# custom-computing-ic/TRPO-Robot-Control

Hardware: AMD Instinct MI355X
Metric: FVP samples/sec + 10-iter CG wall time, armDOF_0 policy (higher is better)
Workload: dtype fp32; 1 GPU; cg10_armDOF_0_N50000; policy=armDOF_0 [15,16,16,3] lttl, samples=50000, samples_per_rank=50000, cg_iters=10, parallelism=dp1 (contiguous sample shards, peer-window all-reduce per FVP), cg_scalars=fp64, fvp_kernel=mfma-mlp3 1x1x1x1 ttl no-mfma

## Files before the change

### trpo-robot-control_amd/csrc/trpo_kernels.hip

```cpp
#include <hip/hip_runtime.h>
#include <rccl/rccl.h>

#include <dlfcn.h>
#include <math.h>
#include <pthread.h>
#include <stdarg.h>
#include <stdint.h>
#include <stdio.h>
#include <stdlib.h>
#include <string.h>
#include <time.h>

#include "trpo_common.h"
#include "trpo_dev.h"

typedef float f4 __attribute__((ext_vector_type(4)));

#define MFMA(a, b, c) __builtin_amdgcn_mfma_f32_16x16x4f32((a), (b), (c), 0, 0, 0)
#define MFMA4(a, b, c) __builtin_amdgcn_mfma_f32_4x4x1f32((a), (b), (c), 0, 0, 0)

struct Pack {
    int T[4];
    int fa[3], fb[3], bi[3], iv, tlen;
    int vfa[3], vb[3], vlen;
// ... 437 lines not shown
            const int a = w / lo, o = w - a * lo;
            const int lane = (o & 15) + 16 * ((a & 15) >> 2);
            return vfa[i] + (((o >> 4) * T[i] + (a >> 4)) * 64 + lane) * 4 + (a & 3);
        }
        if (b >= 0 && b < lo) return vb[i] + b;
    }
    return -1;
}

__device__ __forceinline__ int imap_at(const Net &n, const int (&T)[4], int j) {
    const int k = j >> 8, lane = (j >> 2) & 63, r = j & 3, c = lane & 15, g = lane >> 4;
    int base = 0;
#pragma unroll
    for (int i = 0; i < 3; ++i) {
        const int nt = T[i] * T[i + 1];
        if (k >= base && k < base + nt) {
            const int at = (k - base) / T[i + 1], bt = (k - base) % T[i + 1];
            const int a = 16 * at + 4 * g + r, b = 16 * bt + c;
            return (a < n.L[i] && b < n.L[i + 1]) ? n.woff[i] + a * n.L[i + 1] + b : -1;
        }
        base += nt;
    }
#pragma unroll
    for (int i = 0; i < 3; ++i) {
        if (k >= base && k < base + T[i + 1]) {
            const int b = 16 * (k - base) + 4 * g + r;
            return (c == 0 && b < n.L[i + 1]) ? n.boff[i] + b : -1;
        }
        base += T[i + 1];
    }
    return -1;
}

__device__ __forceinline__ int islot_at(const Net &n, const int (&T)[4], int q) {
    int kw[3], kb[3], k = 0;
#pragma unroll
    for (int i = 0; i < 3; ++i) { kw[i] = k; k += T[i] * T[i + 1]; }
#pragma unroll
    for (int i = 0; i < 3; ++i) { kb[i] = k; k += T[i + 1]; }
#pragma unroll
    for (int i = 0; i < 3; ++i) {
        const int lo = n.L[i + 1], w = q - n.woff[i], b = q - n.boff[i];
        if (w >= 0 && w < n.L[i] * lo) {
            const int a = w / lo, o = w - a * lo;
            return (kw[i] + (a >> 4) * T[i + 1] + (o >> 4)) * 256 + (((a & 15) >> 2) * 16 + (o & 15)) * 4 + (a & 3);
        }
        if (b >= 0 && b < lo) return (kb[i] + (b >> 4)) * 256 + ((b & 15) >> 2) * 64 + (b & 3);
    }
    return -1;
}

__global__ void build_maps_kernel(Net n, Pack pk, int *tmap, int *vmap, int p64) {
    const int e = blockIdx.x * blockDim.x + threadIdx.x;
    if (e < pk.tlen) {
        int m = -1;
        for (int i = 0; i < 3; ++i) {
            if (e >= pk.fa[i] && e < pk.fa[i] + 256 * pk.T[i] * pk.T[i + 1])
                m = map_frag(n, i, e - pk.fa[i], pk.T[i], true, p64 != 0);
            if (i > 0 && e >= pk.fb[i] && e < pk.fb[i] + 256 * pk.T[i] * pk.T[i + 1])
                m = map_frag(n, i, e - pk.fb[i], pk.T[i + 1], false, p64 != 0);
            if (e >= pk.bi[i] && e < pk.bi[i] + 16 * pk.T[i + 1]) {
                const int j = e - pk.bi[i];
                m = j < n.L[i + 1] ? n.boff[i] + j : -1;
            }
        }
        tmap[e] = m;
    }
    if (e < pk.vlen) vmap[e] = vmap_at(n, pk.T, e, p64 != 0);
}

__global__ void build_pslot_kernel(Net n, Pack pk, int *ps, int P) {
    const int q = blockIdx.x * blockDim.x + threadIdx.x;
    const int T[4] = {pk.T[0], pk.T[1], pk.T[2], pk.T[3]};
    if (q < P) ps[q] = pslot_at(n, T, q);
}
__global__ void build_islot_kernel(Net n, Pack pk, int *is, int nw) {
    const int q = blockIdx.x * blockDim.x + threadIdx.x;
    const int T[4] = {pk.T[0], pk.T[1], pk.T[2], pk.T[3]};
    if (q < nw) is[q] = islot_at(n, T, q);
}

__global__ void gather_pack_kernel(void *dst, const double *src, const int *map, int len, int f64) {
    const int e = blockIdx.x * blockDim.x + threadIdx.x;
    if (e < len) {
        const int m = map[e];
        const double v = m >= 0 ? src[m] : 0.0;
        if (f64) reinterpret_cast<double *>(dst)[e] = v;
        else reinterpret_cast<float *>(dst)[e] = (float)v;
    }
}

__global__ void build_imap_kernel(Net n, Pack pk, int *imap, int slab) {
    const int j = blockIdx.x * blockDim.x + threadIdx.x;
    if (j < slab) imap[j] = imap_at(n, pk.T, j);
}

__global__ void iota_kernel(int *v, int len, int valid) {
    const int j = blockIdx.x * blockDim.x + threadIdx.x;
    if (j < len) v[j] = j < valid ? j : -1;
}

__global__ void set_invvar_kernel(void *iv, const double *stdv, int A, int len, int f64) {
    const int j = blockIdx.x * blockDim.x + threadIdx.x;
    if (j < len) {
        const double v = j < A ? 1.0 / stdv[j] / stdv[j] : 0.0;
        if (f64) reinterpret_cast<double *>(iv)[j] = v;
        else reinterpret_cast<float *>(iv)[j] = (float)v;
    }
}

__global__ void obs_pad_kernel(void *dst, const double *src, int n, int npad, int L0, int ld, int f64) {
    const long e = (long)blockIdx.x * blockDim.x + threadIdx.x;
    if (e >= (long)npad * ld) return;
    const int s = (int)(e / ld), k = (int)(e % ld);
    const int q = k & 15, kf = f64 ? (k - q) + (q >> 2) + 4 * (q & 3) : k;
    const double v = (s < n && kf < L0) ? src[(long)s * L0 + kf] : 0.0;
    if (f64) reinterpret_cast<double *>(dst)[e] = v;
    else reinterpret_cast<float *>(dst)[e] = (float)v;
}

__global__ void to_f32_kernel(float *dst, const double *src, int len) {
    const int e = blockIdx.x * blockDim.x + threadIdx.x;
    if (e < len) dst[e] = (float)src[e];
}
__global__ void to_elem_kernel(void *dst, const double *src, long len, int f64) {
    const long e = (long)blockIdx.x * blockDim.x + threadIdx.x;
    if (e >= len) return;
    if (f64) reinterpret_cast<double *>(dst)[e] = src[e];
    else reinterpret_cast<float *>(dst)[e] = (float)src[e];
}


constexpr int SCR_LD = 20;

template <int T0, int T1, int T2, int T3>
struct FastCfg {
    static constexpr int FA0 = 0;
    static constexpr int FA1 = FA0 + 256 * T0 * T1;
    static constexpr int FA2 = FA1 + 256 * T1 * T2;
    static constexpr int FB1 = FA2 + 256 * T2 * T3;
    static constexpr int FB2 = FB1 + 256 * T1 * T2;
    static constexpr int BI0 = FB2 + 256 * T2 * T3;
    static constexpr int BI1 = BI0 + 16 * T1;
    static constexpr int BI2 = BI1 + 16 * T2;
    static constexpr int IV = BI2 + 16 * T3;
    static constexpr int TLEN = IV + 16 * T3;
    static constexpr int VFA0 = 0;
    static constexpr int VFA1 = VFA0 + 256 * T0 * T1;
    static constexpr int VFA2 = VFA1 + 256 * T1 * T2;
    static constexpr int VB0 = VFA2 + 256 * T2 * T3;
    static constexpr int VB1 = VB0 + 16 * T1;
    static constexpr int VB2 = VB1 + 16 * T2;
    static constexpr int VLEN = VB2 + 16 * T3;
    static constexpr int R0 = 16 * (T0 + T1), R1 = 16 * (T1 + T2), R2 = 16 * (T2 + T3);
    static constexpr int ROWS = R0 > R1 ? (R0 > R2 ? R0 : R2) : (R1 > R2 ? R1 : R2);
    static constexpr int SCR = ROWS * 20;
    static constexpr int NACC = 4 * (T0 * T1 + T1 * T2 + T2 * T3 + T1 + T2 + T3);
    static constexpr int SLAB = NACC * 64;
    static constexpr bool REGW = T0 * T1 + T1 * T2 + T2 * T3 <= 3;
    static constexpr int WAVES = 8;
    static constexpr int NT_YC = 1;
    static constexpr int THREADS = 64 * WAVES;
    static constexpr int PMAX = 256 * (T0 * T1 + T1 * T2 + T2 * T3) + 16 * (T1 + T2 + 2 * T3);
    static constexpr int SCRATCH = (WAVES * NT_YC * SCR > 2 * PMAX) ? WAVES * NT_YC * SCR : 2 * PMAX;
    static constexpr int MAIN_BYTES = 4 * (TLEN + VLEN + SCRATCH);
    static constexpr int CAP = MAIN_BYTES > 131072 ? MAIN_BYTES : 131072;
    static constexpr int rw_pick(int w) {
        return w < 1 ? 1 : ((WAVES % w == 0 && w * SLAB * 4 <= CAP) ? w : rw_pick(w - 1));
    }
    static constexpr int RW = rw_pick(WAVES);
    static constexpr int EPT = (SLAB / 4 + THREADS - 1) / THREADS;
    static constexpr int EMAX = (PMAX + THREADS - 1) / THREADS;
    static constexpr int VEMAX = (VLEN + THREADS - 1) / THREADS;
    static constexpr int EMAX_REPLICAS = 4;
    static_assert(NT_YC == 1 || NT_YC == 2, "NT");
    static_assert(WAVES % RW == 0, "RW");
    static int lds_bytes() {
        const int b = 4 * RW * SLAB;
        return MAIN_BYTES > b ? MAIN_BYTES : b;
    }
};

__device__ __forceinline__ float rowsum16(float v) {
    int x = __float_as_int(v);
    v += __int_as_float(__builtin_amdgcn_update_dpp(0, x, 0xB1, 0xF, 0xF, false));
    x = __float_as_int(v);
    v += __int_as_float(__builtin_amdgcn_update_dpp(0, x, 0x4E, 0xF, 0xF, false));
    x = __float_as_int(v);
    v += __int_as_float(__builtin_amdgcn_update_dpp(0, x, 0x124, 0xF, 0xF, false));
    x = __float_as_int(v);
    v += __int_as_float(__builtin_amdgcn_update_dpp(0, x, 0x128, 0xF, 0xF, false));
    return v;
}

__device__ __forceinline__ float rowgroup_sum(float v) {
    const auto h = __builtin_amdgcn_permlane32_swap(__float_as_uint(v), __float_as_uint(v), false, false);
    const float t = __uint_as_float(h[0]) + __uint_as_float(h[1]);
    const auto q = __builtin_amdgcn_permlane16_swap(__float_as_uint(t), __float_as_uint(t), false, false);
    return __uint_as_float(q[0]) + __uint_as_float(q[1]);
}
__device__ __forceinline__ f4 rowgroup_sum4(f4 v) {
    const auto p01 = __builtin_amdgcn_permlane32_swap(__float_as_uint(v[0]), __float_as_uint(v[1]), false, false);
    const auto p23 = __builtin_amdgcn_permlane32_swap(__float_as_uint(v[2]), __float_as_uint(v[3]), false, false);
    const float s01 = __uint_as_float(p01[0]) + __uint_as_float(p01[1]);
    const float s23 = __uint_as_float(p23[0]) + __uint_as_float(p23[1]);
    const auto q = __builtin_amdgcn_permlane16_swap(__float_as_uint(s01), __float_as_uint(s23), false, false);
    const float t = __uint_as_float(q[0]) + __uint_as_float(q[1]);
    const auto h = __builtin_amdgcn_permlane32_swap(__float_as_uint(t), __float_as_uint(t), false, false);
    const auto b02 = __builtin_amdgcn_permlane16_swap(h[0], h[0], false, false);
    const auto b13 = __builtin_amdgcn_permlane16_swap(h[1], h[1], false, false);
    f4 r;
    r[0] = __uint_as_float(b02[0]);
    r[1] = __uint_as_float(b13[0]);
    r[2] = __uint_as_float(b02[1]);
    r[3] = __uint_as_float(b13[1]);
    return r;
}

__device__ __forceinline__ f4 stream_ld(const f4 *p) {
    return *p;
}

__device__ __forceinline__ int scr_off(int row, int chunk) {
    const int q = (row >> 2) & 3;
    return row * 16 + (row >> 2) * 16 + ((chunk ^ ((4 - q) & 3)) << 2);
}
__device__ __forceinline__ void scr_put(float *scr, int row0, f4 t, int c, int g) {
    reinterpret_cast<f4 *>(scr)[(row0 >> 4) * 68 + c + 17 * g] = t;
}
__device__ __forceinline__ f4 scr_get(const float *scr, int row0, int c, int g) {
    const float *p = scr + (row0 >> 4) * 272 + 4 * (4 * g + 17 * (c >> 2)) + (c & 3);
    f4 r;
    r[0] = p[0];
    r[1] = p[4];
    r[2] = p[8];
    r[3] = p[12];
    return r;
}

constexpr int NO_MFMA_RGW2 = 8;
template <int T0, int T1, int T2, int T3, int ACT, int MODE, int QB = 0, int NO = 0>
__global__ void __launch_bounds__((64 * FastCfg<T0, T1, T2, T3>::WAVES))
fvp_mlp3_kernel(const double *__restrict__ k_acc, const double *__restrict__ k_p, const double *__restrict__ k_r,
                const double *__restrict__ k_x, const int *__restrict__ k_pslot, const void *k_q, int k_meta,
                IterArgs A, Net net) {
    constexpr bool FV = MODE != 1;
    constexpr bool YC = MODE == 2 || MODE == 3;
    constexpr int NYC = T1 + T2 + T3;
    using C = FastCfg<T0, T1, T2, T3>;
    constexpr int NT = YC ? C::NT_YC : 1;
    static_assert(!YC || C::REGW, "forward cache only for the small-net kernels");
    extern __shared__ __attribute__((aligned(16))) float lds[];
    __shared__ double sh64[(5 + QB) * 4 * C::WAVES];
    double *shq = reinterpret_cast<double *>(lds + C::TLEN + C::VLEN);
    float *qf = reinterpret_cast<float *>(A.q);
    const float *qfz = reinterpret_cast<const float *>(A.qz);
    const int kPs = k_meta & 0xFFFFF, kR = (k_meta >> 20) & 63, knq = (k_meta >> 26) & 63;
    const float *kq = reinterpret_cast<const float *>(k_q);
    static_assert(C::SCRATCH >= 2 * QCAP * 4 * C::WAVES, "basis-dot scratch");
    float *tw = lds;
    float *vw = lds + C::TLEN;
    const int tid = threadIdx.x, lane = tid & 63, wave = tid >> 6;
    const int c = lane & 15, g = lane >> 4;
    float *scr = lds + C::TLEN + C::VLEN + wave * C::NT_YC * C::SCR;
    const int nwaves = gridDim.x * C::WAVES;
    const int ntiles = A.ntiles, n = A.n;
    const f4 *obs4 = reinterpret_cast<const f4 *>(A.obs4);

    constexpr bool CGK = MODE == 3;
    const bool upd = CGK || (MODE == 0 && A.update != 0);
    const bool ini = !CGK && MODE == 0 && !upd && A.init != 0;
    const bool vnat = !CGK && !upd && !ini && A.v_nat != nullptr;
    constexpr int NT4 = C::TLEN / 4, NALL = CGK ? NT4 : (C::TLEN + C::VLEN) / 4;
    constexpr int PER = (NALL + C::THREADS - 1) / C::THREADS;
    const int skipv = *A.skip;
    f4 st[PER];
    int tile = __builtin_amdgcn_readfirstlane(blockIdx.x * C::WAVES + wave);
    constexpr bool RING = YC;
    constexpr int PFU = RING ? 2 : 1;
    f4 xb[PFU][NT][T0];
    [[maybe_unused]] f4 yb[PFU][NT][YC ? NYC : 1];
    f4(&xn)[T0] = xb[0][0];
    const f4 *yc4 = reinterpret_cast<const f4 *>(A.yc);
    const int a3c = ACT >= 0 ? ((ACT >> 4) & 3) : net.act[3];
    auto load_static = [&]() {
        const f4 *tp4 = reinterpret_cast<const f4 *>(A.tpack);
        const f4 *vp4 = reinterpret_cast<const f4 *>(A.vpack);
#pragma unroll
        for (int k = 0; k < PER; ++k) {
            const int e = min(tid + k * C::THREADS, NALL - 1);
            st[k] = e < NT4 ? tp4[e] : vp4[e - NT4];
        }
#pragma unroll
        for (int t = 0; t < NT; ++t) {
            const int tl = max(0, min(tile + t * nwaves, ntiles - 1));
#pragma unroll
            for (int kt = 0; kt < T0; ++kt) xb[0][t][kt] = obs4[(long)(tl * 16 + c) * (4 * T0) + kt * 4 + g];
            if constexpr (YC) {
#pragma unroll
                for (int k = 0; k < T1 + T2; ++k) yb[0][t][k] = yc4[((long)tl * NYC + k) * 64 + lane];
                if (act_needs_y(a3c))
#pragma unroll
                    for (int k = T1 + T2; k < NYC; ++k) yb[0][t][k] = yc4[((long)tl * NYC + k) * 64 + lane];
            }
        }
    };
    if constexpr (!CGK) load_static();
    constexpr int Tc[4] = {T0, T1, T2, T3};
    constexpr bool PAIR = C::EMAX == 2;
    double pv[C::EMAX], rv[C::EMAX], zv[C::EMAX], xv[C::EMAX];
    int vm[C::VEMAX], ps[C::EMAX];
    CgSt sin = {0.0, 0.0, 0, 0};
// ... 132 lines not shown
            if (ps[e] >= 0) vw[ps[e]] = (float)pv[e];
#pragma unroll
        for (int e = 0; e < C::VEMAX; ++e) {
            const int ve = tid + e * C::THREADS;
            if (ve < C::VLEN && vm[e] < 0) vw[ve] = 0.0f;
        }
        if (blockIdx.x == gridDim.x - 1) {
            double red[1] = {0.0};
#pragma unroll
            for (int e = 0; e < C::EMAX; ++e) red[0] += pv[e] * pv[e];
            block_sums_dpp<1, C::WAVES>(red, sh64);
            const double rr = red[0];
#pragma unroll
            for (int e = 0; e < C::EMAX; ++e) {
                const int q = tid + e * C::THREADS;
                if (q < A.P) {
                    A.p_out[q] = pv[e];
                    A.r_out[q] = pv[e];
                    A.x[q] = 0.0;
                }
            }
            if (A.reorth) qstore<C::EMAX>(qf, A.P, A.Ps, 0, rr, pv, C::THREADS);
            if (tid == 0) {
                A.st_out->rdotr = rr;
                A.st_out->xx = 0.0;
                A.st_out->iter = 0;
                A.hist[0] = rr;
                A.hist[1] = 0.0;
                A.ctl->maxiter = A.init_maxiter;
                A.ctl->resth = A.init_resth;
                A.ctl->rdotr = rr;
                A.ctl->iter = 0;
                A.ctl->orth = 0.0;
                A.ctl->done = (rr < A.init_resth || A.init_maxiter == 0) ? 1 : 0;
            }
        }
    }
    if (upd) {
        #pragma clang fp contract(off)
        double red[5 + QB];
#pragma unroll
        for (int k = 0; k < 5 + QB; ++k) red[k] = 0.0;
#pragma unroll
        for (int e = 0; e < C::EMAX; ++e) {
            const int q = elem_of<PAIR>(e, C::THREADS);
            zv[e] = __builtin_fma(clam, pv[e], q < A.nw ? zv[e] / cn : 2.0 * pv[e]);
            red[0] = __builtin_fma(pv[e], zv[e], red[0]);
            red[1] = __builtin_fma(rv[e], zv[e], red[1]);
            red[2] = __builtin_fma(zv[e], zv[e], red[2]);
            red[3] = __builtin_fma(xv[e], pv[e], red[3]);
            red[4] = __builtin_fma(pv[e], pv[e], red[4]);
#pragma unroll
            for (int i = 0; i < QB; ++i) red[5 + i] = __builtin_fma(qv[i][e], zv[e], red[5 + i]);
        }
        if constexpr (QB == 0) {
            if (A.reorth && A.nq > 0) qdots_stage1<C::EMAX, float, PAIR>(qf, qfz, A.P, A.Ps, A.nq, zv, C::THREADS, shq);
        }
        block_sums_dpp<5 + QB, C::WAVES>(red, sh64);
        const double alpha = sin.rdotr / red[0];
        double cs = 0.0, cr = 0.0;
        if (A.reorth && sin.rdotr > 0.0) {
            const double nrm = sqrt(sin.rdotr), cl = nrm - alpha * (red[1] / nrm);
            cs = cl * cl;
            cr = cl / nrm;
        }
#pragma unroll
        for (int e = 0; e < C::EMAX; ++e) {
            const double r0 = rv[e];
            rv[e] = __builtin_fma(-alpha, zv[e], rv[e]);
            rv[e] = __builtin_fma(-cr, r0, rv[e]);
            xv[e] = __builtin_fma(alpha, pv[e], xv[e]);
        }
        if constexpr (QB > 0) {
#pragma unroll
            for (int i = 0; i < QB; ++i) {
                const double c = -alpha * red[5 + i];
                cs += c * c;
#pragma unroll
                for (int e = 0; e < C::EMAX; ++e) rv[e] = __builtin_fma(-c, qv[i][e], rv[e]);
            }
        } else {
            if (A.reorth && A.nq > 0) cs += qcorrect<C::EMAX, float, PAIR>(qf, qfz, A.P, A.Ps, A.nq, C::THREADS, shq, alpha, rv);
        }
        const double nr = sin.rdotr - 2.0 * alpha * red[1] + alpha * alpha * red[2] - cs;
        const double xn2 = sin.xx + 2.0 * alpha * red[3] + alpha * alpha * red[4];
        const double beta = nr / sin.rdotr;
#pragma unroll
        for (int e = 0; e < C::EMAX; ++e) {
            const int q = elem_of<PAIR>(e, C::THREADS);
            pv[e] = __builtin_fma(beta, pv[e], rv[e]);
            if (q < A.P && blockIdx.x == 0) {
                A.p_out[q] = pv[e];
                A.r_out[q] = rv[e];
                A.x[q] = xv[e];
            }
        }
        const int it = sin.iter + 1;
        const int done = (nr < cth || it >= cmax) ? 1 : 0;
        if (blockIdx.x == 0 && A.reorth) qstore<C::EMAX, float, PAIR>(qf, A.P, A.Ps, it, nr, rv, C::THREADS);
        if (blockIdx.x == 0 && tid == 0) {
            A.st_out->rdotr = nr;
            A.st_out->xx = xn2;
            A.st_out->iter = it;
            A.hist[2 * it] = nr;
            A.hist[2 * it + 1] = sqrt(xn2);
            A.ctl->rdotr = nr;
            A.ctl->iter = it;
            A.ctl->done = done;
            note_orth(&A.ctl->orth, cs, nr);
            if (it <= CG_AMAX) A.ctl->alpha[it - 1] = alpha;
        }
        if (done) return;
#pragma unroll
        for (int e = 0; e < C::EMAX; ++e)
            if (ps[e] >= 0) vw[ps[e]] = (float)pv[e];
#pragma unroll
        for (int e = 0; e < C::VEMAX; ++e) {
            const int ve = tid + e * C::THREADS;
            if (ve < C::VLEN && vm[e] < 0) vw[ve] = 0.0f;
        }
    }
    if constexpr (CGK) stage_static();
    __syncthreads();
    [[maybe_unused]] int jslot[C::EMAX];
    if constexpr (C::RW == C::WAVES) {
        if (A.islot) {
#pragma unroll
            for (int e = 0; e < C::EMAX; ++e) jslot[e] = A.islot[min(tid + e * C::THREADS, A.nw - 1)];
        }
    }
    [[maybe_unused]] bool first_tile = true;

    const int a1 = ACT >= 0 ? (ACT & 3) : net.act[1];
    const int a2 = ACT >= 0 ? ((ACT >> 2) & 3) : net.act[2];
    const int a3 = ACT >= 0 ? ((ACT >> 4) & 3) : net.act[3];
    const bool y3_needed = act_needs_y(a3);
    f4 *ycs = (MODE == 0 && C::REGW) ? reinterpret_cast<f4 *>(A.yc) : nullptr;
    const f4 *TW = reinterpret_cast<const f4 *>(tw);
    const f4 *VW = reinterpret_cast<const f4 *>(vw);

    const f4 zero4 = {0.f, 0.f, 0.f, 0.f};
    f4 rFA0 = zero4, rVFA0 = zero4, rFA1 = zero4, rVFA1 = zero4, rFA2 = zero4, rVFA2 = zero4, rFB1 = zero4,
       rFB2 = zero4;
    if constexpr (C::REGW) {
        rFA0 = TW[C::FA0 / 4 + lane];
        rVFA0 = VW[C::VFA0 / 4 + lane];
        rFA1 = TW[C::FA1 / 4 + lane];
        rVFA1 = VW[C::VFA1 / 4 + lane];
        rFA2 = TW[C::FA2 / 4 + lane];
        rVFA2 = VW[C::VFA2 / 4 + lane];
        rFB1 = TW[C::FB1 / 4 + lane];
        rFB2 = TW[C::FB2 / 4 + lane];
    }
#define WLD(REG, EXPR) (C::REGW ? (REG) : (EXPR))
    constexpr int NOUT = NO & 7;
    static_assert(NO == 0 || (T3 == 1 && NOUT >= 1 && NOUT <= 4), "narrow output layer");
    constexpr int NOA = NOUT ? NOUT : 1;
    constexpr bool NOV = NOUT && !(NO & NO_MFMA_RGW2);
    [[maybe_unused]] f4 nFA2[T2], nVFA2[T2], w2n[T2][4];
    [[maybe_unused]] f4 nb2 = zero4, nvb2 = zero4, niv = zero4;
    [[maybe_unused]] float acc2[T2][4][NOA], sb3n[NOA];
    if constexpr (NO) {
        const int lp = (c & 3) + 16 * g;
#pragma unroll
        for (int kt = 0; kt < T2; ++kt) {
            nFA2[kt] = TW[C::FA2 / 4 + kt * 64 + lp];
            nVFA2[kt] = FV ? VW[C::VFA2 / 4 + kt * 64 + lp] : zero4;
#pragma unroll
            for (int r = 0; r < 4; ++r) w2n[kt][r] = TW[C::FB2 / 4 + kt * 64 + 4 * g + r];
#pragma unroll
            for (int r = 0; r < 4; ++r)
#pragma unroll
                for (int o = 0; o < NOA; ++o) acc2[kt][r][o] = 0.0f;
        }
        nb2 = g == 0 ? TW[C::BI2 / 4] : zero4;
        nvb2 = (FV && g == 0) ? VW[C::VB2 / 4] : zero4;
        niv = TW[C::IV / 4];
#pragma unroll
        for (int o = 0; o < NOA; ++o) sb3n[o] = 0.0f;
    }
    f4 accW0[T0][T1], accW1[T1][T2], accW2[T2][T3];
    f4 sB1[T1], sB2[T2], sB3[T3];
#pragma unroll
    for (int a = 0; a < T0; ++a)
#pragma unroll
        for (int b = 0; b < T1; ++b) accW0[a][b] = zero4;
#pragma unroll
    for (int a = 0; a < T1; ++a)
#pragma unroll
        for (int b = 0; b < T2; ++b) accW1[a][b] = zero4;
#pragma unroll
    for (int a = 0; a < T2; ++a)
#pragma unroll
        for (int b = 0; b < T3; ++b) accW2[a][b] = zero4;
#pragma unroll
    for (int a = 0; a < T1; ++a) sB1[a] = zero4;
#pragma unroll
    for (int a = 0; a < T2; ++a) sB2[a] = zero4;
#pragma unroll
    for (int a = 0; a < T3; ++a) sB3[a] = zero4;

    [[maybe_unused]] const int pf_xoff = (c * (4 * T0) + g) * 16, pf_yoff = lane * 16;
    auto tile_step = [&](const int tile, const f4 (&x0)[NT][T0], const f4 (&ycur)[NT][YC ? NYC : 1],
                         const bool (&live)[NT]) __attribute__((always_inline)) {
        f4 y1[NT][T1], r1[NT][T1];
#pragma unroll
        for (int ot = 0; ot < T1; ++ot) {
            const f4 b0 = TW[C::BI0 / 4 + ot * 4 + g], vb0 = VW[C::VB0 / 4 + ot * 4 + g];
            f4 a[NT], ra[NT];
#pragma unroll
            for (int t = 0; t < NT; ++t) {
                a[t] = b0;
                ra[t] = vb0;
            }
#pragma unroll
            for (int kt = 0; kt < T0; ++kt) {
                const f4 w = WLD(rFA0, TW[C::FA0 / 4 + (ot * T0 + kt) * 64 + lane]);
                const f4 u = FV ? WLD(rVFA0, VW[C::VFA0 / 4 + (ot * T0 + kt) * 64 + lane]) : zero4;
#pragma unroll
                for (int s = 0; s < 4; ++s)
#pragma unroll
                    for (int t = 0; t < NT; ++t) {
                        if constexpr (!YC) a[t] = MFMA(w[s], x0[t][kt][s], a[t]);
                        if constexpr (FV) ra[t] = MFMA(u[s], x0[t][kt][s], ra[t]);
                    }
            }
            if constexpr (YC) {
#pragma unroll
                for (int t = 0; t < NT; ++t) {
                    y1[t][ot] = ycur[t][ot];
                    r1[t][ot] = act_r4(a1, y1[t][ot], ra[t]);
                }
            } else {
#pragma unroll
                for (int t = 0; t < NT; ++t) y1[t][ot] = act_fwd(a1, a[t], ra[t], r1[t][ot]);
                if (ycs) ycs[((long)tile * NYC + ot) * 64 + lane] = y1[0][ot];
            }
        }
        f4 y2[NT][T2], r2[NT][T2];
#pragma unroll
        for (int ot = 0; ot < T2; ++ot) {
            const f4 b1 = TW[C::BI1 / 4 + ot * 4 + g], vb1 = VW[C::VB1 / 4 + ot * 4 + g];
            f4 a[NT], ra[NT], rb[NT];
#pragma unroll
            for (int t = 0; t < NT; ++t) {
                a[t] = b1;
                ra[t] = vb1;
                rb[t] = zero4;
            }
#pragma unroll
            for (int kt = 0; kt < T1; ++kt) {
                const f4 w = WLD(rFA1, TW[C::FA1 / 4 + (ot * T1 + kt) * 64 + lane]);
                const f4 u = FV ? WLD(rVFA1, VW[C::VFA1 / 4 + (ot * T1 + kt) * 64 + lane]) : zero4;
#pragma unroll
                for (int s = 0; s < 4; ++s)
#pragma unroll
                    for (int t = 0; t < NT; ++t) {
                        if constexpr (!YC) a[t] = MFMA(w[s], y1[t][kt][s], a[t]);
                        if constexpr (FV) {
                            ra[t] = MFMA(w[s], r1[t][kt][s], ra[t]);
                            rb[t] = MFMA(u[s], y1[t][kt][s], rb[t]);
                        }
                    }
            }
            if constexpr (YC) {
#pragma unroll
                for (int t = 0; t < NT; ++t) {
                    y2[t][ot] = ycur[t][T1 + ot];
                    r2[t][ot] = act_r4(a2, y2[t][ot], ra[t] + rb[t]);
                }
            } else {
#pragma unroll
                for (int t = 0; t < NT; ++t) y2[t][ot] = act_fwd(a2, a[t], ra[t] + rb[t], r2[t][ot]);
                if (ycs) ycs[((long)tile * NYC + T1 + ot) * 64 + lane] = y2[0][ot];
            }
        }
        f4 g3[NT][T3];
        if constexpr (NO) {
            f4 a[NT], ra[NT], rb[NT];
#pragma unroll
            for (int t = 0; t < NT; ++t) {
                a[t] = nb2;
                ra[t] = nvb2;
                rb[t] = zero4;
            }
#pragma unroll
            for (int kt = 0; kt < T2; ++kt)
#pragma unroll
                for (int s = 0; s < 4; ++s)
#pragma unroll
                    for (int t = 0; t < NT; ++t) {
                        if (!YC && y3_needed) a[t] = MFMA4(nFA2[kt][s], y2[t][kt][s], a[t]);
                        if constexpr (FV) {
                            ra[t] = MFMA4(nFA2[kt][s], r2[t][kt][s], ra[t]);
                            rb[t] = MFMA4(nVFA2[kt][s], y2[t][kt][s], rb[t]);
                        }
                    }
#pragma unroll
            for (int t = 0; t < NT; ++t) {
                const f4 rx = FV ? rowgroup_sum4(ra[t] + rb[t]) : zero4;
                f4 r3, gg, y3;
                if constexpr (YC) {
                    y3 = y3_needed ? ycur[t][T1 + T2] : zero4;
                    r3 = act_r4(a3, y3, rx);
                } else {
                    y3 = act_fwd(a3, y3_needed ? rowgroup_sum4(a[t]) : zero4, rx, r3);
                    if (ycs && y3_needed) ycs[((long)tile * NYC + T1 + T2) * 64 + lane] = y3;
                }
                if constexpr (FV) {
                    gg = act_bwd(a3, y3, r3 * niv);
                } else {
                    const int tt = min(tile + t * nwaves, ntiles - 1);
                    const f4 dm = reinterpret_cast<const f4 *>(A.pg_d4)[(long)(tt * 16 + c) * 4];
                    const float adv = A.pg_adv[tt * 16 + c];
                    gg = act_bwd(a3, y3, (adv * dm) * reinterpret_cast<const f4 *>(A.pg_iv4)[0]);
                }
                g3[t][0] = live[t] ? gg : zero4;
                if constexpr (NOV) {
#pragma unroll
                    for (int o = 0; o < NOA; ++o) sb3n[o] += g3[t][0][o];
                }
            }
        } else
#pragma unroll
        for (int ot = 0; ot < T3; ++ot) {
            const f4 b2 = TW[C::BI2 / 4 + ot * 4 + g], vb2 = VW[C::VB2 / 4 + ot * 4 + g];
            const f4 iv = TW[C::IV / 4 + ot * 4 + g];
            f4 a[NT], ra[NT], rb[NT];
#pragma unroll
            for (int t = 0; t < NT; ++t) {
                a[t] = b2;
                ra[t] = vb2;
                rb[t] = zero4;
            }
#pragma unroll
            for (int kt = 0; kt < T2; ++kt) {
                const f4 w = WLD(rFA2, TW[C::FA2 / 4 + (ot * T2 + kt) * 64 + lane]);
                const f4 u = FV ? WLD(rVFA2, VW[C::VFA2 / 4 + (ot * T2 + kt) * 64 + lane]) : zero4;
#pragma unroll
                for (int s = 0; s < 4; ++s)
#pragma unroll
                    for (int t = 0; t < NT; ++t) {
                        if (!YC && y3_needed) a[t] = MFMA(w[s], y2[t][kt][s], a[t]);
                        if constexpr (FV) {
                            ra[t] = MFMA(w[s], r2[t][kt][s], ra[t]);
                            rb[t] = MFMA(u[s], y2[t][kt][s], rb[t]);
                        }
                    }
            }
#pragma unroll
            for (int t = 0; t < NT; ++t) {
                f4 r3, gg, y3;
                if constexpr (YC) {
                    y3 = y3_needed ? ycur[t][T1 + T2 + ot] : zero4;
                    r3 = act_r4(a3, y3, ra[t] + rb[t]);
                } else {
                    y3 = act_fwd(a3, a[t], ra[t] + rb[t], r3);
                    if (ycs && y3_needed) ycs[((long)tile * NYC + T1 + T2 + ot) * 64 + lane] = y3;
                }
                if constexpr (FV) {
                    gg = act_bwd(a3, y3, r3 * iv);
                } else {
                    const int tt = min(tile + t * nwaves, ntiles - 1);
                    const f4 dm = reinterpret_cast<const f4 *>(A.pg_d4)[(long)(tt * 16 + c) * (4 * T3) + ot * 4 + g];
                    const float adv = A.pg_adv[tt * 16 + c];
                    gg = act_bwd(a3, y3, (adv * dm) * reinterpret_cast<const f4 *>(A.pg_iv4)[ot * 4 + g]);
                }
                g3[t][ot] = live[t] ? gg : zero4;
                sB3[ot] += g3[t][ot];
            }
        }
        [[maybe_unused]] f4 g3m[NT][T3];
        if constexpr (NO && !NOV) {
#pragma unroll
            for (int t = 0; t < NT; ++t) {
                g3m[t][0] = g == 0 ? g3[t][0] : zero4;
                sB3[0] += g3m[t][0];
            }
        }
        if constexpr (NOV) {
#pragma unroll
            for (int t = 0; t < NT; ++t)
#pragma unroll
                for (int kt = 0; kt < T2; ++kt)
#pragma unroll
                    for (int r = 0; r < 4; ++r)
#pragma unroll
                        for (int o = 0; o < NOA; ++o)
                            acc2[kt][r][o] = fmaf(y2[t][kt][r], g3[t][0][o], acc2[kt][r][o]);
        } else {
#pragma unroll
        for (int t = 0; t < NT; ++t) {
            float *sc = scr + t * C::SCR;
#pragma unroll
            for (int i = 0; i < T2; ++i) scr_put(sc, 16 * i, y2[t][i], c, g);
#pragma unroll
            for (int i = 0; i < T3; ++i) scr_put(sc, 16 * (T2 + i), NO ? g3m[t][i] : g3[t][i], c, g);
        }
#pragma unroll
        for (int t = 0; t < NT; ++t) {
            const float *sc = scr + t * C::SCR;
            f4 gb[T3];
#pragma unroll
            for (int i = 0; i < T3; ++i) gb[i] = scr_get(sc, 16 * (T2 + i), c, g);
#pragma unroll
            for (int at = 0; at < T2; ++at) {
                const f4 ya = scr_get(sc, 16 * at, c, g);
#pragma unroll
                for (int bt = 0; bt < T3; ++bt)
#pragma unroll
                    for (int s = 0; s < 4; ++s) accW2[at][bt] = MFMA(ya[s], gb[bt][s], accW2[at][bt]);
            }
        }
        }
        f4 g2[NT][T2];
#pragma unroll
        for (int it = 0; it < T2; ++it) {
            f4 a[NT];
#pragma unroll
            for (int t = 0; t < NT; ++t) a[t] = zero4;
            if constexpr (NO) {
#pragma unroll
                for (int t = 0; t < NT; ++t)
#pragma unroll
                    for (int r = 0; r < 4; ++r)
#pragma unroll
                        for (int o = 0; o < NOA; ++o) a[t][r] = fmaf(w2n[it][r][o], g3[t][0][o], a[t][r]);
            } else
#pragma unroll
            for (int kt = 0; kt < T3; ++kt) {
                const f4 w = WLD(rFB2, TW[C::FB2 / 4 + (it * T3 + kt) * 64 + lane]);
#pragma unroll
                for (int s = 0; s < 4; ++s)
#pragma unroll
                    for (int t = 0; t < NT; ++t) a[t] = MFMA(w[s], g3[t][kt][s], a[t]);
            }
#pragma unroll
            for (int t = 0; t < NT; ++t) {
                g2[t][it] = act_bwd(a2, y2[t][it], a[t]);
                sB2[it] += g2[t][it];
            }
        }
#pragma unroll
        for (int t = 0; t < NT; ++t) {
            float *sc = scr + t * C::SCR;
#pragma unroll
            for (int i = 0; i < T1; ++i) scr_put(sc, 16 * i, y1[t][i], c, g);
#pragma unroll
            for (int i = 0; i < T2; ++i) scr_put(sc, 16 * (T1 + i), g2[t][i], c, g);
        }
#pragma unroll
        for (int t = 0; t < NT; ++t) {
            const float *sc = scr + t * C::SCR;
            f4 gb[T2];
#pragma unroll
            for (int i = 0; i < T2; ++i) gb[i] = scr_get(sc, 16 * (T1 + i), c, g);
#pragma unroll
            for (int at = 0; at < T1; ++at) {
                const f4 ya = scr_get(sc, 16 * at, c, g);
#pragma unroll
                for (int bt = 0; bt < T2; ++bt)
#pragma unroll
                    for (int s = 0; s < 4; ++s) accW1[at][bt] = MFMA(ya[s], gb[bt][s], accW1[at][bt]);
            }
        }
        f4 g1[NT][T1];
#pragma unroll
        for (int it = 0; it < T1; ++it) {
            f4 a[NT];
#pragma unroll
            for (int t = 0; t < NT; ++t) a[t] = zero4;
#pragma unroll
            for (int kt = 0; kt < T2; ++kt) {
                const f4 w = WLD(rFB1, TW[C::FB1 / 4 + (it * T2 + kt) * 64 + lane]);
#pragma unroll
                for (int s = 0; s < 4; ++s)
#pragma unroll
                    for (int t = 0; t < NT; ++t) a[t] = MFMA(w[s], g2[t][kt][s], a[t]);
            }
#pragma unroll
            for (int t = 0; t < NT; ++t) {
                g1[t][it] = act_bwd(a1, y1[t][it], a[t]);
                sB1[it] += g1[t][it];
            }
        }
#pragma unroll
        for (int t = 0; t < NT; ++t) {
            float *sc = scr + t * C::SCR;
#pragma unroll
            for (int i = 0; i < T0; ++i) scr_put(sc, 16 * i, x0[t][i], c, g);
#pragma unroll
            for (int i = 0; i < T1; ++i) scr_put(sc, 16 * (T0 + i), g1[t][i], c, g);
        }
#pragma unroll
        for (int t = 0; t < NT; ++t) {
            const float *sc = scr + t * C::SCR;
            f4 gb[T1];
#pragma unroll
            for (int i = 0; i < T1; ++i) gb[i] = scr_get(sc, 16 * (T0 + i), c, g);
#pragma unroll
            for (int at = 0; at < T0; ++at) {
                const f4 ya = scr_get(sc, 16 * at, c, g);
#pragma unroll
                for (int bt = 0; bt < T1; ++bt)
#pragma unroll
                    for (int s = 0; s < 4; ++s) accW0[at][bt] = MFMA(ya[s], gb[bt][s], accW0[at][bt]);
            }
        }
    };
    if constexpr (RING) {
        while (tile < ntiles) {
#pragma unroll
            for (int j = 0; j < PFU; ++j) {
                if (tile >= ntiles) break;
                const int sl = (j + 1) % PFU;
#pragma unroll
                for (int t = 0; t < NT; ++t) {
                    const int tn = min(tile + (NT + t) * nwaves, ntiles - 1);
                    const auto rx = __builtin_amdgcn_make_buffer_rsrc((void *)(obs4 + (long)tn * (16 * 4 * T0)), 0,
                                                                      16 * 64 * T0, 0x00020000);
#pragma unroll
                    for (int kt = 0; kt < T0; ++kt)
                        xb[sl][t][kt] =
                            __builtin_bit_cast(f4, __builtin_amdgcn_raw_buffer_load_b128(rx, pf_xoff + kt * 64, 0, 0));
                    const auto ry = __builtin_amdgcn_make_buffer_rsrc((void *)(yc4 + (long)tn * (NYC * 64)), 0,
                                                                      NYC * 1024, 0x00020000);
#pragma unroll
                    for (int k = 0; k < T1 + T2; ++k)
                        yb[sl][t][k] =
                            __builtin_bit_cast(f4, __builtin_amdgcn_raw_buffer_load_b128(ry, pf_yoff + k * 1024, 0, 0));
                    if (y3_needed)
#pragma unroll
                        for (int k = T1 + T2; k < NYC; ++k)
                            yb[sl][t][k] = __builtin_bit_cast(
                                f4, __builtin_amdgcn_raw_buffer_load_b128(ry, pf_yoff + k * 1024, 0, 0));
                }
                __builtin_amdgcn_sched_barrier(0);
                bool live[NT];
#pragma unroll
                for (int t = 0; t < NT; ++t) live[t] = (tile + t * nwaves) * 16 + c < n;
                tile_step(tile, xb[j], yb[j], live);
                tile += NT * nwaves;
            }
        }
    } else {
        static_assert(NT == 1, "one tile per trip outside the cached-forward ring");
        for (; tile < ntiles; tile += nwaves) {
            f4 x0[1][T0];
            const f4 ycur[1][1] = {{zero4}};
            const bool live[1] = {tile * 16 + c < n};
#pragma unroll
            for (int kt = 0; kt < T0; ++kt) x0[0][kt] = xn[kt];
            {
                const int tn = min(tile + nwaves, ntiles - 1);
                const auto rx = __builtin_amdgcn_make_buffer_rsrc((void *)(obs4 + (long)tn * (16 * 4 * T0)), 0,
                                                                  16 * 64 * T0, 0x00020000);
#pragma unroll
                for (int kt = 0; kt < T0; ++kt)
                    xn[kt] = __builtin_bit_cast(f4, __builtin_amdgcn_raw_buffer_load_b128(rx, pf_xoff + kt * 64, 0, 0));
                __builtin_amdgcn_sched_barrier(0);
            }
            tile_step(tile, x0, ycur, live);
        }
    }

#pragma unroll
    for (int a = 0; a < T1; ++a)
#pragma unroll
        for (int r = 0; r < 4; ++r) sB1[a][r] = rowsum16(sB1[a][r]);
#pragma unroll
    for (int a = 0; a < T2; ++a)
#pragma unroll
        for (int r = 0; r < 4; ++r) sB2[a][r] = rowsum16(sB2[a][r]);
    if constexpr (NOV) {
#pragma unroll
        for (int o = 0; o < NOA; ++o) sb3n[o] = rowsum16(sb3n[o]);
#pragma unroll
        for (int kt = 0; kt < T2; ++kt)
#pragma unroll
            for (int r = 0; r < 4; ++r) {
                float v = 0.0f;
#pragma unroll
                for (int o = 0; o < NOA; ++o) {
                    const float t = rowsum16(acc2[kt][r][o]);
                    v = c == o ? t : v;
                }
                accW2[kt][0][r] = v;
            }
#pragma unroll
        for (int r = 0; r < 4; ++r) sB3[0][r] = (g == 0 && r < NOA) ? sb3n[r < NOA ? r : 0] : 0.0f;
    } else {
#pragma unroll
    for (int a = 0; a < T3; ++a)
#pragma unroll
        for (int r = 0; r < 4; ++r) sB3[a][r] = rowsum16(sB3[a][r]);
    }
    f4 acc[C::NACC / 4];
    {
        int k = 0;
#pragma unroll
        for (int a = 0; a < T0; ++a)
#pragma unroll
            for (int b = 0; b < T1; ++b) acc[k++] = accW0[a][b];
#pragma unroll
        for (int a = 0; a < T1; ++a)
#pragma unroll
            for (int b = 0; b < T2; ++b) acc[k++] = accW1[a][b];
#pragma unroll
        for (int a = 0; a < T2; ++a)
#pragma unroll
            for (int b = 0; b < T3; ++b) acc[k++] = accW2[a][b];
#pragma unroll
        for (int a = 0; a < T1; ++a) acc[k++] = sB1[a];
#pragma unroll
        for (int a = 0; a < T2; ++a) acc[k++] = sB2[a];
#pragma unroll
        for (int a = 0; a < T3; ++a) acc[k++] = sB3[a];
    }
    f4 *red = reinterpret_cast<f4 *>(lds);
    if constexpr (C::RW == C::WAVES) {
        if (A.acc_out) {
            __syncthreads();
#pragma unroll
            for (int k = 0; k < C::NACC / 4; ++k) red[wave * (C::SLAB / 4) + k * 64 + lane] = acc[k];
            __syncthreads();
            double *dst = A.acc_out + (long)(blockIdx.x % A.R_out) * A.Ps;
#pragma unroll
            for (int e = 0; e < C::EMAX; ++e) {
                const int q = tid + e * C::THREADS;
                if (q < A.nw) {
                    const int j = A.islot ? jslot[e] : islot_at(net, Tc, q);
                    float t = 0.0f;
#pragma unroll
                    for (int w = 0; w < C::WAVES; ++w) t += lds[w * C::SLAB + j];
                    unsafeAtomicAdd(dst + q, (double)t);
                }
            }
            if (blockIdx.x == 0)
                for (int e = tid; e < A.zero_len; e += C::THREADS) A.acc_zero[e] = 0.0;
            return;
        }
    }
    f4 part[C::EPT];
#pragma unroll
    for (int j = 0; j < C::EPT; ++j) part[j] = zero4;
#pragma unroll
    for (int w0 = 0; w0 < C::WAVES; w0 += C::RW) {
        __syncthreads();
        if (wave >= w0 && wave < w0 + C::RW) {
#pragma unroll
            for (int k = 0; k < C::NACC / 4; ++k) red[(wave - w0) * (C::SLAB / 4) + k * 64 + lane] = acc[k];
        }
        __syncthreads();
#pragma unroll
        for (int j = 0; j < C::EPT; ++j) {
            const int e = tid + j * C::THREADS;
            if (e < C::SLAB / 4) {
#pragma unroll
                for (int w = 0; w < C::RW; ++w) part[j] += red[w * (C::SLAB / 4) + e];
            }
// ... 3497 lines not shown
```

Measured before the change: 5.429 billion FVP samples/s.

## Defer weight-gradient MFMAs and split LDS scratch regions in register-weight FVP kernel

For the small register-resident-weight configuration, the scratch LDS is split into separate per-layer regions so forward activations and backward gradients can be transposed through LDS early. All three weight-gradient outer-product MFMA chains are then batched at the end of the tile step. Bias vectors are hoisted into registers, and the independent V·y (rb) products are computed before the dependent chains, with sched_barriers to order memory ops. The aim is to break serial LDS write/read/MFMA dependencies and interleave independent work. The cost is more live registers and a larger scratch footprint.

```diff
diff --git a/trpo-robot-control_amd/csrc/trpo_kernels.hip b/trpo-robot-control_amd/csrc/trpo_kernels.hip
--- a/trpo-robot-control_amd/csrc/trpo_kernels.hip
+++ b/trpo-robot-control_amd/csrc/trpo_kernels.hip
@@ -613,12 +613,18 @@
     static constexpr int VB1 = VB0 + 16 * T1;
     static constexpr int VB2 = VB1 + 16 * T2;
     static constexpr int VLEN = VB2 + 16 * T3;
+    static constexpr bool REGW = T0 * T1 + T1 * T2 + T2 * T3 <= 3;
+    static constexpr int SCR_SLOT = 272;
     static constexpr int R0 = 16 * (T0 + T1), R1 = 16 * (T1 + T2), R2 = 16 * (T2 + T3);
     static constexpr int ROWS = R0 > R1 ? (R0 > R2 ? R0 : R2) : (R1 > R2 ? R1 : R2);
-    static constexpr int SCR = ROWS * 20;
+    static constexpr int SCR2 = 0;
+    static constexpr int SCR1 = REGW ? SCR2 + SCR_SLOT * (T2 + T3) : 0;
+    static constexpr int SCR0 = REGW ? SCR1 + SCR_SLOT * (T1 + T2) : 0;
+    static constexpr int SCR = REGW ? SCR0 + SCR_SLOT * (T0 + T1) : ROWS * 20;
+    static_assert(SCR_SLOT % 4 == 0 && SCR_SLOT >= 4 * (15 + 17 * 3 + 1), "scr_put slot: f4 index c + 17 g");
+    static_assert(SCR >= SCR_SLOT * (ROWS / 16), "a contraction's operand pair fits its region");
     static constexpr int NACC = 4 * (T0 * T1 + T1 * T2 + T2 * T3 + T1 + T2 + T3);
     static constexpr int SLAB = NACC * 64;
-    static constexpr bool REGW = T0 * T1 + T1 * T2 + T2 * T3 <= 3;
     static constexpr int WAVES = 8;
     static constexpr int NT_YC = 1;
     static constexpr int THREADS = 64 * WAVES;
@@ -1057,6 +1063,27 @@
         rFB1 = TW[C::FB1 / 4 + lane];
         rFB2 = TW[C::FB2 / 4 + lane];
     }
+    [[maybe_unused]] f4 hB0[T1], hVB0[T1], hB1[T2], hVB1[T2], hB2[T3], hVB2[T3], hIV[T3];
+    if constexpr (C::REGW) {
+#pragma unroll
+        for (int ot = 0; ot < T1; ++ot) {
+            hB0[ot] = TW[C::BI0 / 4 + ot * 4 + g];
+            hVB0[ot] = VW[C::VB0 / 4 + ot * 4 + g];
+        }
+#pragma unroll
+        for (int ot = 0; ot < T2; ++ot) {
+            hB1[ot] = TW[C::BI1 / 4 + ot * 4 + g];
+            hVB1[ot] = VW[C::VB1 / 4 + ot * 4 + g];
+        }
+        if constexpr (NO == 0) {
+#pragma unroll
+            for (int ot = 0; ot < T3; ++ot) {
+                hB2[ot] = TW[C::BI2 / 4 + ot * 4 + g];
+                hVB2[ot] = VW[C::VB2 / 4 + ot * 4 + g];
+                hIV[ot] = TW[C::IV / 4 + ot * 4 + g];
+            }
+        }
+    }
 #define WLD(REG, EXPR) (C::REGW ? (REG) : (EXPR))
     constexpr int NOUT = NO & 7;
     static_assert(NO == 0 || (T3 == 1 && NOUT >= 1 && NOUT <= 4), "narrow output layer");
@@ -1106,12 +1133,31 @@
     for (int a = 0; a < T3; ++a) sB3[a] = zero4;
 
     [[maybe_unused]] const int pf_xoff = (c * (4 * T0) + g) * 16, pf_yoff = lane * 16;
+    constexpr bool DEFER = C::REGW, RBFIRST = C::REGW;
+    constexpr int SCHED_MEM = 0x4 | 0x10 | 0x80;
     auto tile_step = [&](const int tile, const f4 (&x0)[NT][T0], const f4 (&ycur)[NT][YC ? NYC : 1],
                          const bool (&live)[NT]) __attribute__((always_inline)) {
+        [[maybe_unused]] f4 ya2[NT][T2], ya1[NT][T1], ya0[NT][T0], gb2[NT][T3], gb1[NT][T2], gb0[NT][T1];
+        auto tput = [&](int t, int region, int slot, const f4 v) __attribute__((always_inline)) {
+            scr_put(scr + t * C::SCR + region, 16 * slot, v, c, g);
+        };
+        auto tget = [&](int t, int region, int slot) __attribute__((always_inline)) {
+            return scr_get(scr + t * C::SCR + region, 16 * slot, c, g);
+        };
+        if constexpr (DEFER) {
+#pragma unroll
+            for (int t = 0; t < NT; ++t) {
+#pragma unroll
+                for (int i = 0; i < T0; ++i) tput(t, C::SCR0, i, x0[t][i]);
+#pragma unroll
+                for (int i = 0; i < T0; ++i) ya0[t][i] = tget(t, C::SCR0, i);
+            }
+        }
         f4 y1[NT][T1], r1[NT][T1];
+        [[maybe_unused]] f4 ra0[NT][T1];
 #pragma unroll
         for (int ot = 0; ot < T1; ++ot) {
-            const f4 b0 = TW[C::BI0 / 4 + ot * 4 + g], vb0 = VW[C::VB0 / 4 + ot * 4 + g];
+            const f4 b0 = WLD(hB0[ot], TW[C::BI0 / 4 + ot * 4 + g]), vb0 = WLD(hVB0[ot], VW[C::VB0 / 4 + ot * 4 + g]);
             f4 a[NT], ra[NT];
 #pragma unroll
             for (int t = 0; t < NT; ++t) {
@@ -1134,18 +1180,54 @@
 #pragma unroll
                 for (int t = 0; t < NT; ++t) {
                     y1[t][ot] = ycur[t][ot];
-                    r1[t][ot] = act_r4(a1, y1[t][ot], ra[t]);
+                    ra0[t][ot] = ra[t];
                 }
             } else {
 #pragma unroll
                 for (int t = 0; t < NT; ++t) y1[t][ot] = act_fwd(a1, a[t], ra[t], r1[t][ot]);
                 if (ycs) ycs[((long)tile * NYC + ot) * 64 + lane] = y1[0][ot];
-            }
+                if constexpr (DEFER) {
+#pragma unroll
+                    for (int t = 0; t < NT; ++t) {
+                        tput(t, C::SCR1, ot, y1[t][ot]);
+                        ya1[t][ot] = tget(t, C::SCR1, ot);
+                    }
+                }
+            }
+        }
+        [[maybe_unused]] f4 rb1[NT][T2];
+        if constexpr (YC) {
+#pragma unroll
+            for (int t = 0; t < NT; ++t) {
+#pragma unroll
+                for (int i = 0; i < T1; ++i) tput(t, C::SCR1, i, y1[t][i]);
+#pragma unroll
+                for (int i = 0; i < T1; ++i) ya1[t][i] = tget(t, C::SCR1, i);
+            }
+#pragma unroll
+            for (int ot = 0; ot < T2; ++ot) {
+#pragma unroll
+                for (int t = 0; t < NT; ++t) rb1[t][ot] = zero4;
+#pragma unroll
+                for (int kt = 0; kt < T1; ++kt) {
+                    const f4 u = WLD(rVFA1, VW[C::VFA1 / 4 + (ot * T1 + kt) * 64 + lane]);
+#pragma unroll
+                    for (int s = 0; s < 4; ++s)
+#pragma unroll
+                        for (int t = 0; t < NT; ++t) rb1[t][ot] = MFMA(u[s], y1[t][kt][s], rb1[t][ot]);
+                }
+            }
+            __builtin_amdgcn_sched_barrier(SCHED_MEM);
+#pragma unroll
+            for (int ot = 0; ot < T1; ++ot)
+#pragma unroll
+                for (int t = 0; t < NT; ++t) r1[t][ot] = act_r4(a1, y1[t][ot], ra0[t][ot]);
         }
         f4 y2[NT][T2], r2[NT][T2];
+        [[maybe_unused]] f4 ra1[NT][T2];
 #pragma unroll
         for (int ot = 0; ot < T2; ++ot) {
-            const f4 b1 = TW[C::BI1 / 4 + ot * 4 + g], vb1 = VW[C::VB1 / 4 + ot * 4 + g];
+            const f4 b1 = WLD(hB1[ot], TW[C::BI1 / 4 + ot * 4 + g]), vb1 = WLD(hVB1[ot], VW[C::VB1 / 4 + ot * 4 + g]);
             f4 a[NT], ra[NT], rb[NT];
 #pragma unroll
             for (int t = 0; t < NT; ++t) {
@@ -1153,10 +1235,20 @@
                 ra[t] = vb1;
                 rb[t] = zero4;
             }
+            if constexpr (FV && !YC && RBFIRST) {
+#pragma unroll
+                for (int kt = 0; kt < T1; ++kt) {
+                    const f4 u = WLD(rVFA1, VW[C::VFA1 / 4 + (ot * T1 + kt) * 64 + lane]);
+#pragma unroll
+                    for (int s = 0; s < 4; ++s)
+#pragma unroll
+                        for (int t = 0; t < NT; ++t) rb[t] = MFMA(u[s], y1[t][kt][s], rb[t]);
+                }
+            }
 #pragma unroll
             for (int kt = 0; kt < T1; ++kt) {
                 const f4 w = WLD(rFA1, TW[C::FA1 / 4 + (ot * T1 + kt) * 64 + lane]);
-                const f4 u = FV ? WLD(rVFA1, VW[C::VFA1 / 4 + (ot * T1 + kt) * 64 + lane]) : zero4;
+                const f4 u = (FV && !RBFIRST) ? WLD(rVFA1, VW[C::VFA1 / 4 + (ot * T1 + kt) * 64 + lane]) : zero4;
 #pragma unroll
                 for (int s = 0; s < 4; ++s)
 #pragma unroll
@@ -1164,7 +1256,7 @@
                         if constexpr (!YC) a[t] = MFMA(w[s], y1[t][kt][s], a[t]);
                         if constexpr (FV) {
                             ra[t] = MFMA(w[s], r1[t][kt][s], ra[t]);
-                            rb[t] = MFMA(u[s], y1[t][kt][s], rb[t]);
+                            if constexpr (!RBFIRST) rb[t] = MFMA(u[s], y1[t][kt][s], rb[t]);
                         }
                     }
             }
@@ -1172,13 +1264,53 @@
 #pragma unroll
                 for (int t = 0; t < NT; ++t) {
                     y2[t][ot] = ycur[t][T1 + ot];
-                    r2[t][ot] = act_r4(a2, y2[t][ot], ra[t] + rb[t]);
+                    ra1[t][ot] = ra[t];
                 }
             } else {
 #pragma unroll
                 for (int t = 0; t < NT; ++t) y2[t][ot] = act_fwd(a2, a[t], ra[t] + rb[t], r2[t][ot]);
                 if (ycs) ycs[((long)tile * NYC + T1 + ot) * 64 + lane] = y2[0][ot];
-            }
+                if constexpr (DEFER && !NOV) {
+#pragma unroll
+                    for (int t = 0; t < NT; ++t) {
+                        tput(t, C::SCR2, ot, y2[t][ot]);
+                        ya2[t][ot] = tget(t, C::SCR2, ot);
+                    }
+                }
+            }
+        }
+        [[maybe_unused]] f4 rb2[NT][T3];
+        if constexpr (YC) {
+            if constexpr (!NOV) {
+#pragma unroll
+                for (int t = 0; t < NT; ++t) {
+#pragma unroll
+                    for (int i = 0; i < T2; ++i) tput(t, C::SCR2, i, y2[t][i]);
+#pragma unroll
+                    for (int i = 0; i < T2; ++i) ya2[t][i] = tget(t, C::SCR2, i);
+                }
+            }
+#pragma unroll
+            for (int ot = 0; ot < T3; ++ot) {
+#pragma unroll
+                for (int t = 0; t < NT; ++t) rb2[t][ot] = zero4;
+#pragma unroll
+                for (int kt = 0; kt < T2; ++kt) {
+                    const f4 u = NO ? nVFA2[kt] : WLD(rVFA2, VW[C::VFA2 / 4 + (ot * T2 + kt) * 64 + lane]);
+#pragma unroll
+                    for (int s = 0; s < 4; ++s)
+#pragma unroll
+                        for (int t = 0; t < NT; ++t) {
+                            if constexpr (NO) rb2[t][ot] = MFMA4(u[s], y2[t][kt][s], rb2[t][ot]);
+                            else rb2[t][ot] = MFMA(u[s], y2[t][kt][s], rb2[t][ot]);
+                        }
+                }
+            }
+            __builtin_amdgcn_sched_barrier(SCHED_MEM);
+#pragma unroll
+            for (int ot = 0; ot < T2; ++ot)
+#pragma unroll
+                for (int t = 0; t < NT; ++t) r2[t][ot] = act_r4(a2, y2[t][ot], ra1[t][ot] + rb1[t][ot]);
         }
         f4 g3[NT][T3];
         if constexpr (NO) {
@@ -1188,6 +1320,15 @@
                 a[t] = nb2;
                 ra[t] = nvb2;
                 rb[t] = zero4;
+                if constexpr (YC) rb[t] = rb2[t][0];
+            }
+            if constexpr (FV && !YC) {
+#pragma unroll
+                for (int kt = 0; kt < T2; ++kt)
+#pragma unroll
+                    for (int s = 0; s < 4; ++s)
+#pragma unroll
+                        for (int t = 0; t < NT; ++t) rb[t] = MFMA4(nVFA2[kt][s], y2[t][kt][s], rb[t]);
             }
 #pragma unroll
             for (int kt = 0; kt < T2; ++kt)
@@ -1196,10 +1337,7 @@
 #pragma unroll
                     for (int t = 0; t < NT; ++t) {
                         if (!YC && y3_needed) a[t] = MFMA4(nFA2[kt][s], y2[t][kt][s], a[t]);
-                        if constexpr (FV) {
-                            ra[t] = MFMA4(nFA2[kt][s], r2[t][kt][s], ra[t]);
-                            rb[t] = MFMA4(nVFA2[kt][s], y2[t][kt][s], rb[t]);
-                        }
+                        if constexpr (FV) ra[t] = MFMA4(nFA2[kt][s], r2[t][kt][s], ra[t]);
                     }
 #pragma unroll
             for (int t = 0; t < NT; ++t) {
@@ -1229,19 +1367,30 @@
         } else
 #pragma unroll
         for (int ot = 0; ot < T3; ++ot) {
-            const f4 b2 = TW[C::BI2 / 4 + ot * 4 + g], vb2 = VW[C::VB2 / 4 + ot * 4 + g];
-            const f4 iv = TW[C::IV / 4 + ot * 4 + g];
+            const f4 b2 = WLD(hB2[ot], TW[C::BI2 / 4 + ot * 4 + g]), vb2 = WLD(hVB2[ot], VW[C::VB2 / 4 + ot * 4 + g]);
+            const f4 iv = WLD(hIV[ot], TW[C::IV / 4 + ot * 4 + g]);
             f4 a[NT], ra[NT], rb[NT];
 #pragma unroll
             for (int t = 0; t < NT; ++t) {
                 a[t] = b2;
                 ra[t] = vb2;
                 rb[t] = zero4;
+                if constexpr (YC) rb[t] = rb2[t][ot];
+            }
+            if constexpr (FV && !YC && RBFIRST) {
+#pragma unroll
+                for (int kt = 0; kt < T2; ++kt) {
+                    const f4 u = WLD(rVFA2, VW[C::VFA2 / 4 + (ot * T2 + kt) * 64 + lane]);
+#pragma unroll
+                    for (int s = 0; s < 4; ++s)
+#pragma unroll
+                        for (int t = 0; t < NT; ++t) rb[t] = MFMA(u[s], y2[t][kt][s], rb[t]);
+                }
             }
 #pragma unroll
             for (int kt = 0; kt < T2; ++kt) {
                 const f4 w = WLD(rFA2, TW[C::FA2 / 4 + (ot * T2 + kt) * 64 + lane]);
-                const f4 u = FV ? WLD(rVFA2, VW[C::VFA2 / 4 + (ot * T2 + kt) * 64 + lane]) : zero4;
+                const f4 u = (FV && !RBFIRST) ? WLD(rVFA2, VW[C::VFA2 / 4 + (ot * T2 + kt) * 64 + lane]) : zero4;
 #pragma unroll
                 for (int s = 0; s < 4; ++s)
 #pragma unroll
@@ -1249,7 +1398,7 @@
                         if (!YC && y3_needed) a[t] = MFMA(w[s], y2[t][kt][s], a[t]);
                         if constexpr (FV) {
                             ra[t] = MFMA(w[s], r2[t][kt][s], ra[t]);
-                            rb[t] = MFMA(u[s], y2[t][kt][s], rb[t]);
+                            if constexpr (!RBFIRST) rb[t] = MFMA(u[s], y2[t][kt][s], rb[t]);
                         }
                     }
             }
@@ -1293,6 +1442,14 @@
 #pragma unroll
                         for (int o = 0; o < NOA; ++o)
                             acc2[kt][r][o] = fmaf(y2[t][kt][r], g3[t][0][o], acc2[kt][r][o]);
+        } else if constexpr (DEFER) {
+#pragma unroll
+            for (int t = 0; t < NT; ++t)
+#pragma unroll
+                for (int i = 0; i < T3; ++i) {
+                    tput(t, C::SCR2, T2 + i, NO ? g3m[t][i] : g3[t][i]);
+                    gb2[t][i] = tget(t, C::SCR2, T2 + i);
+                }
         } else {
 #pragma unroll
         for (int t = 0; t < NT; ++t) {
@@ -1346,6 +1503,15 @@
                 sB2[it] += g2[t][it];
             }
         }
+        if constexpr (DEFER) {
+#pragma unroll
+            for (int t = 0; t < NT; ++t)
+#pragma unroll
+                for (int i = 0; i < T2; ++i) {
+                    tput(t, C::SCR1, T1 + i, g2[t][i]);
+                    gb1[t][i] = tget(t, C::SCR1, T1 + i);
+                }
+        } else {
 #pragma unroll
         for (int t = 0; t < NT; ++t) {
             float *sc = scr + t * C::SCR;
@@ -1369,6 +1535,7 @@
                     for (int s = 0; s < 4; ++s) accW1[at][bt] = MFMA(ya[s], gb[bt][s], accW1[at][bt]);
             }
         }
+        }
         f4 g1[NT][T1];
 #pragma unroll
         for (int it = 0; it < T1; ++it) {
@@ -1389,6 +1556,38 @@
                 sB1[it] += g1[t][it];
             }
         }
+        if constexpr (DEFER) {
+#pragma unroll
+            for (int t = 0; t < NT; ++t)
+#pragma unroll
+                for (int i = 0; i < T1; ++i) {
+                    tput(t, C::SCR0, T0 + i, g1[t][i]);
+                    gb0[t][i] = tget(t, C::SCR0, T0 + i);
+                }
+            __builtin_amdgcn_sched_barrier(0);
+#pragma unroll
+            for (int t = 0; t < NT; ++t)
+#pragma unroll
+                for (int s = 0; s < 4; ++s) {
+                    if constexpr (!NOV) {
+#pragma unroll
+                        for (int at = 0; at < T2; ++at)
+#pragma unroll
+                            for (int bt = 0; bt < T3; ++bt)
+                                accW2[at][bt] = MFMA(ya2[t][at][s], gb2[t][bt][s], accW2[at][bt]);
+                    }
+#pragma unroll
+                    for (int at = 0; at < T1; ++at)
+#pragma unroll
+                        for (int bt = 0; bt < T2; ++bt)
+                            accW1[at][bt] = MFMA(ya1[t][at][s], gb1[t][bt][s], accW1[at][bt]);
+#pragma unroll
+                    for (int at = 0; at < T0; ++at)
+#pragma unroll
+                        for (int bt = 0; bt < T1; ++bt)
+                            accW0[at][bt] = MFMA(ya0[t][at][s], gb0[t][bt][s], accW0[at][bt]);
+                }
+        } else {
 #pragma unroll
         for (int t = 0; t < NT; ++t) {
             float *sc = scr + t * C::SCR;
@@ -1411,6 +1610,7 @@
 #pragma unroll
                     for (int s = 0; s < 4; ++s) accW0[at][bt] = MFMA(ya[s], gb[bt][s], accW0[at][bt]);
             }
+        }
         }
     };
     if constexpr (RING) {
```

New measurement: 5.486 billion FVP samples/s, median of 6. 1.0% higher.
